# fasion-image-generator-project/discogan_modernized

Measured on AMD Instinct MI355X. Metric: images/sec per DiscoGAN train step, higher is better.
Workload: dtype f32x3; 1 GPU; tops2hanbok discogan image_size=512 batch_size=32 per GPU (BASELINE configs[3]); D,G,G cycle, fwd+bwd+Adam, dead backward work skipped; fp32-accurate conv products on the bf16 matrix path: every fp32 operand carried as three bf16 planes (24 significand bits), exact bf16 x bf16 products, fp32 accumulation (no operand rounding); image_size=512, global_batch=32, parallelism=dp1, hipgraph=True, hip_streams=2, allreduce_overlap=False

## Files before the change

discogan_modernized_amd/csrc/edge.hip:

```cpp
#include "dg_common.h"
#include <type_traits>

__device__ float dg_zero_edge[64];

__device__ __forceinline__ int tap_of(int parity, int d) {
    if (parity == 0) return d == 0 ? 1 : (d == -1 ? 3 : -1);
    return d == 0 ? 2 : (d == 1 ? 0 : -1);
}

__global__ __launch_bounds__(256) void c3_dgrad_valu_kernel(const float* __restrict__ dy, const float* __restrict__ w,
                                                            float* __restrict__ dx, int N, int H, int W, int K,
                                                            int lgHo, int lgWo, int act) {
    const int Ho = H >> 1, Wo = W >> 1;
    const long nquad = (long)N * Ho * Wo;
    const long q = (long)blockIdx.x * 256 + threadIdx.x;
    if (q >= nquad) return;
    const int b = (int)(q & (Wo - 1)), a = (int)((q >> lgWo) & (Ho - 1)), n = (int)(q >> (lgWo + lgHo));
    float acc[3][2][2];
#pragma unroll
    for (int c = 0; c < 3; ++c) acc[c][0][0] = acc[c][0][1] = acc[c][1][0] = acc[c][1][1] = 0.f;
    const float* base = dy + ((long)(n * Ho + a) * Wo + b) * K;
    for (int k0 = 0; k0 < K; k0 += 4) {
        f32x4 g[3][3];
#pragma unroll
// ... 260 lines not shown
                }
        } else if constexpr (MF16) {
#pragma unroll
            for (int st = 0; st < 2; ++st)
#pragma unroll
                for (int g = 0; g < 2; ++g)
#pragma unroll
                    for (int blk = 0; blk < 3; ++blk)
                        acc[g][blk] = __builtin_amdgcn_mfma_f32_16x16x32_bf16(__builtin_bit_cast(bf16x8_d, areg[S][g][st]), breg16[blk][st],
                                                                              acc[g][blk], 0, 0, 0);
        } else
#pragma unroll
        for (int s = 0; s < 16; ++s)
#pragma unroll
            for (int g = 0; g < 2; ++g)
#pragma unroll
                for (int blk = 0; blk < 3; ++blk)
                {
                    float av;
                    if constexpr (IN16) {
                        const float fv = areg[S][g][s >> 3][(s >> 1) & 3];
                        const unsigned wv = __float_as_uint(fv);
                        av = __builtin_bit_cast(float, (s & 1) ? (wv & 0xffff0000u) : (wv << 16));
                    } else {
                        av = areg[S][g][s >> 2][s & 3];
                    }
                    acc[g][blk] = __builtin_amdgcn_mfma_f32_16x16x4f32(av, breg[blk][s], acc[g][blk], 0, 0, 0);
                }
        __syncthreads();
#pragma unroll
        for (int g = 0; g < 2; ++g)
#pragma unroll
            for (int blk = 0; blk < 3; ++blk)
#pragma unroll
                for (int j = 0; j < 4; ++j) Ps[((wave + 4 * g) * CS_PC + 4 * kq + j) * CS_LDP + blk * 16 + p] = acc[g][blk][j];
        __syncthreads();
        for (int e = tid; e < 3 * 2 * CS_TR * 2 * CS_TC; e += 256) {
            const int xx = e % (2 * CS_TC), yy = (e / (2 * CS_TC)) % (2 * CS_TR), c = e / (4 * CS_TR * CS_TC);
            const int y = 2 * a0 + yy, x = 2 * b0 + xx;
            const int ph = yy & 1, pw = xx & 1, la = (yy >> 1) + 1, lb = (xx >> 1) + 1;
            const int ra2 = la - 1 + 2 * ph, rr1 = 1 + ph, rr2 = 3 - 3 * ph;
            const int cb2 = lb - 1 + 2 * pw, ss1 = 1 + pw, ss2 = 3 - 3 * pw;
            const float* pc = Ps + c * 16;
            float v = pc[(la * CS_PC + lb) * CS_LDP + rr1 * 4 + ss1] + pc[(la * CS_PC + cb2) * CS_LDP + rr1 * 4 + ss2] +
                      pc[(ra2 * CS_PC + lb) * CS_LDP + rr2 * 4 + ss1] + pc[(ra2 * CS_PC + cb2) * CS_LDP + rr2 * 4 + ss2];
            if (act == DG_ACT_SIGMOID) v = 1.f / (1.f + expf(-v));
            if (y < H && x < W) dx[((long)(n * 3 + c) * H + y) * W + x] = v;
        }
        apply_act(S ^ 1);
    };
    for (int t = blockIdx.x; t < ntiles; t += 2 * gridDim.x) {
        tile(std::integral_constant<int, 0>{}, t);
        if (t + (int)gridDim.x < ntiles) tile(std::integral_constant<int, 1>{}, t + gridDim.x);
    }
}

extern "C" size_t dg_c3_dgrad_workspace_bytes(int K) { return K == CD_K ? (size_t)CD_NK * 16 * sizeof(float) : 0; }
static int c3_dgrad_run(int groups, const float* const* dy_nhwc, int dy_bf16, const float* const* w, float* const* dx_nchw, int N, int H, int W, int K,
                        int act, void* ws, size_t ws_bytes, dg_stream_t stream, const void* act_out = nullptr, float slope = 0.f);
extern "C" int dg_conv4x4s2_c3_dgrad(const float* dy_nhwc, const float* w, float* dx_nchw, int N, int H, int W, int K,
                                     int act, void* ws, size_t ws_bytes, dg_stream_t stream) {
    return c3_dgrad_run(1, &dy_nhwc, 0, &w, &dx_nchw, N, H, W, K, act, ws, ws_bytes, stream);
}
extern "C" int dg_conv4x4s2_c3_dgrad_t(const void* dy_nhwc, int dy_bf16, const float* w, float* dx_nchw, int N, int H, int W, int K,
                                       int act, void* ws, size_t ws_bytes, dg_stream_t stream) {
    const float* dyp = (const float*)dy_nhwc;
    return c3_dgrad_run(1, &dyp, dy_bf16, &w, &dx_nchw, N, H, W, K, act, ws, ws_bytes, stream);
}
extern "C" int dg_conv4x4s2_c3_dgrad_p(const void* dy_nhwc, int dy_bf16, const float* w, float* dx_nchw, int N, int H, int W, int K,
                                       int act, int prec, void* ws, size_t ws_bytes, dg_stream_t stream) {
    DG_CHECK_ARG(prec >= DG_PREC_DEFAULT && prec <= DG_PREC_F32X3, "dg_conv4x4s2_c3_dgrad_p: prec=%d", prec);
    DgPrecScope scope(prec);
    const float* dyp = (const float*)dy_nhwc;
    return c3_dgrad_run(1, &dyp, dy_bf16, &w, &dx_nchw, N, H, W, K, act, ws, ws_bytes, stream);
}
static bool c3_dgrad_scatter_fits(int N, int H, int W, int K, int dy_bf16) {
    return K == CD_K && N >= 1 && (long)N * (H / 2) * (W / 2) * CD_K * (dy_bf16 ? 2 : 4) < (1L << 31);
}
extern "C" int dg_c3_dgrad_act_ok(int N, int H, int W, int K, int dy_bf16) {
    return c3_dgrad_scatter_fits(N, H, W, K, dy_bf16) && dg_get_option(DG_OPT_KT) != 16 ? 1 : 0;
}
extern "C" int dg_conv4x4s2_c3_dgrad_act_p(const void* dy_nhwc, int dy_bf16, const void* act_out, int in_act, float slope, const float* w, float* dx_nchw,
                                           int N, int H, int W, int K, int act, int prec, void* ws, size_t ws_bytes, dg_stream_t stream) {
    DG_CHECK_ARG(prec >= DG_PREC_DEFAULT && prec <= DG_PREC_F32X3, "dg_conv4x4s2_c3_dgrad_act_p: prec=%d", prec);
    DG_CHECK_ARG(act_out && in_act == DG_ACT_LEAKY, "dg_conv4x4s2_c3_dgrad_act_p: needs the saved output of a fused LeakyReLU (in_act=%d)", in_act);
    DG_CHECK_ARG(dg_c3_dgrad_act_ok(N, H, W, K, dy_bf16), "dg_conv4x4s2_c3_dgrad_act_p: the fused form is the scatter kernel (K == 64, dy under 2^31 bytes, option kt != 16)");
    DgPrecScope scope(prec);
    const float* dyp = (const float*)dy_nhwc;
    return c3_dgrad_run(1, &dyp, dy_bf16, &w, &dx_nchw, N, H, W, K, act, ws, ws_bytes, stream, act_out, slope);
}
extern "C" int dg_conv4x4s2_c3_dgrad_g(int groups, const float* const* dy_nhwc, const float* const* w, float* const* dx_nchw, int N, int H, int W, int K,
                                       int act, int prec, dg_stream_t stream) {
    DG_CHECK_ARG(groups >= 1 && groups <= DG_MAX_GROUPS && dy_nhwc && w && dx_nchw, "dg_conv4x4s2_c3_dgrad_g: bad group / null table");
    DG_CHECK_ARG(prec >= DG_PREC_DEFAULT && prec <= DG_PREC_F32X3, "dg_conv4x4s2_c3_dgrad_g: prec=%d", prec);
    DG_CHECK_ARG(K == CD_K && dg_get_option(DG_OPT_KT) != 16, "dg_conv4x4s2_c3_dgrad_g: the grouped form is the scatter kernel (K == 64)");
    DgPrecScope scope(prec);
    return c3_dgrad_run(groups, dy_nhwc, 0, w, dx_nchw, N, H, W, K, act, nullptr, 0, stream);
}
static int c3_dgrad_run(int groups, const float* const* dy_tab, int dy_bf16, const float* const* w_tab, float* const* dx_tab, int N, int H, int W, int K,
                        int act, void* ws, size_t ws_bytes, dg_stream_t stream, const void* act_out, float slope) {
    DG_CHECK_ARG(act_out == nullptr || groups == 1, "dg_conv4x4s2_c3_dgrad: the fused activation backward takes one problem");
    for (int i = 0; i < groups; ++i) DG_CHECK_ARG(dy_tab[i] && w_tab[i] && dx_tab[i], "dg_conv4x4s2_c3_dgrad: null pointer");
    const float* dy_nhwc = dy_tab[0];
    const float* w = w_tab[0];
    float* dx_nchw = dx_tab[0];
    DG_CHECK_ARG(!dy_bf16 || (K == CD_K && dg_get_option(DG_OPT_KT) != 16), "dg_conv4x4s2_c3_dgrad_t: a bf16 dy needs K == 64 (scatter form)");
    DG_CHECK_ARG(N >= 1 && K >= 4 && K % 4 == 0, "dg_conv4x4s2_c3_dgrad: bad N/K (%d,%d)", N, K);
    DG_CHECK_ARG(dg_is_pow2(H) && dg_is_pow2(W) && H >= 2 && W >= 2, "dg_conv4x4s2_c3_dgrad: H,W must be powers of two");
    DG_CHECK_ARG(act == DG_ACT_NONE || act == DG_ACT_SIGMOID, "dg_conv4x4s2_c3_dgrad: bad act %d", act);
    DG_CHECK_ARG((long)N * 3 * H * W < (1L << 31), "dg_conv4x4s2_c3_dgrad: tensor too large");
    hipStream_t st = (hipStream_t)stream;
    const int Ho = H / 2, Wo = W / 2;
    if (c3_dgrad_scatter_fits(N, H, W, K, dy_bf16)) {
        if (dg_get_option(DG_OPT_KT) != 16) {
            const int tiles_r = (Ho + CS_TR - 1) / CS_TR, tiles_c = (Wo + CS_TC - 1) / CS_TC;
            const long ntiles = (long)N * tiles_r * tiles_c;
            DG_CHECK_ARG(ntiles < (1L << 30), "dg_conv4x4s2_c3_dgrad: too many tiles");
            const dim3 grid((unsigned)(ntiles < 512 ? ntiles : 512), groups);
            const DgPtrs pd = dg_ptrs((const void* const*)dy_tab, groups), pw = dg_ptrs((const void* const*)w_tab, groups),
                         px = dg_ptrs((const void* const*)dx_tab, groups);
            const DgPtrs pa = dg_ptrs1(act_out ? act_out : (const void*)dy_tab[0]);
            const unsigned dyb = (unsigned)((long)N * Ho * Wo * CD_K * (dy_bf16 ? 2 : 4));
#define C3_SCATTER(...) hipLaunchKernelGGL((c3_dgrad_scatter_kernel<__VA_ARGS__>), grid, dim3(256), 0, st, pd, pw, px, N, H, W, act, tiles_r, tiles_c, (int)ntiles, dyb, pa, slope)
            if (dy_bf16 && dg_cur_prec() == 1) {
                if (act_out) C3_SCATTER(true, true, false, true); else C3_SCATTER(true, true);
            } else if (dy_bf16) {
                if (act_out) C3_SCATTER(true, false, false, true); else C3_SCATTER(true, false);
            } else if (dg_cur_prec() == 2) {
                if (act_out) C3_SCATTER(false, false, true, true); else C3_SCATTER(false, false, true);
            } else {
                if (act_out) C3_SCATTER(false, false, false, true); else C3_SCATTER(false, false);
            }
#undef C3_SCATTER
            DG_CHECK_LAUNCH("c3_dgrad_scatter");
            return DG_OK;
        }
        DG_CHECK_ARG(groups == 1 && !act_out, "dg_conv4x4s2_c3_dgrad: the gather form takes one problem and no fused activation backward");
        DG_CHECK_ARG(!dy_bf16, "dg_conv4x4s2_c3_dgrad: the gather form reads an fp32 dy (a bf16 dy needs the scatter form)");
        const int tiles_r = (Ho + CD_TR - 1) / CD_TR, tiles_c = (Wo + CD_TC - 1) / CD_TC;
        const long ntiles = (long)N * tiles_r * tiles_c;
        DG_CHECK_ARG(ntiles < (1L << 31), "dg_conv4x4s2_c3_dgrad: too many tiles");
        if (ws == nullptr || ws_bytes < dg_c3_dgrad_workspace_bytes(K))
            return dg_fail(DG_ERR_WORKSPACE, "dg_conv4x4s2_c3_dgrad: workspace %zu < %zu", ws_bytes, dg_c3_dgrad_workspace_bytes(K));
        hipLaunchKernelGGL(c3_wq_build_kernel, dim3((CD_NK * 16 + 255) / 256), dim3(256), 0, st, w, (float*)ws);
        DG_CHECK_LAUNCH("c3_wq_build");
        const int grid = (int)(ntiles < 512 ? ntiles : 512);
        hipLaunchKernelGGL(c3_dgrad_mfma_kernel, dim3(grid), dim3(256), 0, st, dy_nhwc, (const float*)ws, dx_nchw, N, H, W, act,
                           tiles_r, tiles_c, (int)ntiles);
        DG_CHECK_LAUNCH("c3_dgrad_mfma");
        return DG_OK;
    }
    DG_CHECK_ARG(groups == 1 && !act_out, "dg_conv4x4s2_c3_dgrad: the VALU form takes one problem and no fused activation backward");
    DG_CHECK_ARG(!dy_bf16, "dg_conv4x4s2_c3_dgrad: the VALU form reads an fp32 dy (a bf16 dy of %ld bytes is past the scatter form's 2^31)",
                 (long)N * Ho * Wo * K * 2);
    const long nquad = (long)N * Ho * Wo;
    hipLaunchKernelGGL(c3_dgrad_valu_kernel, dim3((unsigned)((nquad + 255) / 256)), dim3(256), 0, st, dy_nhwc, w,
                       dx_nchw, N, H, W, K, dg_ilog2(Ho), dg_ilog2(Wo), act);
    DG_CHECK_LAUNCH("c3_dgrad_valu");
    return DG_OK;
}

#define CF_K 64
#define CF_S 24
template <int ACT, bool OUT16>
__global__ __launch_bounds__(256, 2) void c3_fwd_mfma_kernel(const DgPtrs xs, const DgPtrs ws_, const DgPtrs ys, int N, int H, int W, int lgHo, int lgWo,
                                                             long npix, int ngroups, float slope, int xbytes) {
    const float* __restrict__ x = dg_pick<const float>(xs, blockIdx.y);
    const float* __restrict__ w = dg_pick<const float>(ws_, blockIdx.y);
    float* __restrict__ y = dg_pick<float>(ys, blockIdx.y);
    const int lane = threadIdx.x & 63;
    const int p = lane & 31, h = lane >> 5;
    const int Ho = H >> 1, Wo = W >> 1;
    const int wave = blockIdx.x * 4 + (threadIdx.x >> 6), nwaves = gridDim.x * 4;
    const float* const zp = dg_zero_edge;
    __shared__ float wS[CF_K * 49];
    for (int e = threadIdx.x; e < CF_K * 48; e += 256) wS[(e / 48) * 49 + e % 48] = w[e];
    __syncthreads();
    float wb[2][CF_S];
#pragma unroll
    for (int nb = 0; nb < 2; ++nb)
#pragma unroll
        for (int s = 0; s < CF_S; ++s) {
// ... 524 lines not shown
        u32x4_w ev, od;
#pragma unroll
        for (int u = 0; u < 4; ++u) {
            ev[u] = __builtin_amdgcn_perm(w8[2 * u + 1], w8[2 * u], 0x05040100u);
            od[u] = __builtin_amdgcn_perm(w8[2 * u + 1], w8[2 * u], 0x07060302u);
        }
        fa[0] = __builtin_bit_cast(bf16x8_w, ev);
        fa[1] = __builtin_bit_cast(bf16x8_w, od);
#pragma unroll
        for (int jn = 0; jn < 2; ++jn) {
            f32x8_w t8;
#pragma unroll
            for (int t = 0; t < 8; ++t) t8[t] = fb[set][jn][t];
            fbv[jn] = __builtin_convertvector(t8, bf16x8_w);
        }
#pragma unroll
        for (int i = 0; i < 2; ++i)
#pragma unroll
            for (int jn = 0; jn < 2; ++jn) acc[i][jn] = __builtin_amdgcn_mfma_f32_32x32x16_bf16(fa[i], fbv[jn], acc[i][jn], 0, 0, 0);
    };
    load_batch(0, p_begin);
    for (long p0 = p_begin; p0 < p_end; p0 += 32) {
        load_batch(1, p0 + 16);
        mma_batch(0);
        load_batch(0, p0 + 32);
        mma_batch(1);
    }
    __shared__ float slabS[4][64 * 48];
#pragma unroll
    for (int i = 0; i < 2; ++i)
#pragma unroll
        for (int r = 0; r < 16; ++r) {
            const int rho = (r & 3) + 8 * (r >> 2) + 4 * lh;
            const int k = 2 * rho + i;
#pragma unroll
            for (int jn = 0; jn < 2; ++jn) {
                const int j = jn * 32 + l31;
                if (j < 48) slabS[wave][k * 48 + j] = acc[i][jn][r];
            }
        }
    __syncthreads();
    float* slab = part + ((long)blockIdx.x * K + kg * 64) * 48;
    for (int e = tid; e < 64 * 48; e += 256) slab[e] = ((slabS[0][e] + slabS[1][e]) + slabS[2][e]) + slabS[3][e];
}

#define CWL_WOMAX 256
template <typename F>
__device__ __forceinline__ void c3_static_for4(F&& f) {
    f(std::integral_constant<int, 0>{});
    f(std::integral_constant<int, 1>{});
    f(std::integral_constant<int, 2>{});
    f(std::integral_constant<int, 3>{});
}
template <bool FACT, bool X3 = false>
__global__ __launch_bounds__(256, X3 ? 1 : 2) void c3_wgrad_lds_kernel(const DgPtrs dys, const DgPtrs xs, const DgPtrs parts, int N, int H, int W, int K,
                                                              long npix, int rows_per_wg, const DgPtrs act_outs, float slope) {
    const float* __restrict__ dy = dg_pick<const float>(dys, blockIdx.z);
    const float* __restrict__ x = dg_pick<const float>(xs, blockIdx.z);
    float* __restrict__ part = dg_pick<float>(parts, blockIdx.z);
    const float* __restrict__ act_out = dg_pick<const float>(act_outs, blockIdx.z);
    constexpr int ROWE = CWL_WOMAX + 8;
    typedef typename std::conditional<X3, float, __bf16>::type ET;
    __shared__ __attribute__((aligned(16))) ET img[2][4][12][ROWE];
    const int tid = threadIdx.x, lane = tid & 63, wave = tid >> 6;
    const int l31 = lane & 31, lh = lane >> 5;
    const int Ho = H >> 1, Wo = W >> 1;
    const int kg = blockIdx.y;
    f32x16 acc[2][2];
#pragma unroll
    for (int i = 0; i < 2; ++i)
#pragma unroll
        for (int j = 0; j < 2; ++j)
#pragma unroll
            for (int r = 0; r < 16; ++r) acc[i][j][r] = 0.f;
    int jrow[2], jarr[2];
    bool jok[2];
#pragma unroll
    for (int jn = 0; jn < 2; ++jn) {
        const int j = jn * 32 + l31;
        jok[jn] = j < 48;
        const int jj = jok[jn] ? j : 0;
        jarr[jn] = jj & 3;
        jrow[jn] = (jj >> 4) * 4 + ((jj >> 2) & 3);
    }
    const int nrows = N * Ho;
    const int u0 = blockIdx.x * rows_per_wg, u1 = min(nrows, u0 + rows_per_wg);
    constexpr int BIG = 0x40000000;
    constexpr int EB = X3 ? 4 : 2;
    const __amdgpu_buffer_rsrc_t rdy = __builtin_amdgcn_make_buffer_rsrc((void*)dy, 0, (int)(npix * K * EB), 0x00020000);
    const __amdgpu_buffer_rsrc_t rao = __builtin_amdgcn_make_buffer_rsrc((void*)(FACT ? act_out : dy), 0, (int)(npix * K * EB), 0x00020000);
    auto bload = [](const __amdgpu_buffer_rsrc_t& r, int off) -> unsigned {
        return (unsigned)__builtin_amdgcn_raw_buffer_load_b32(r, off, 0, 0);
    };
    typedef float f32x2_w __attribute__((ext_vector_type(2)));
    auto bload2 = [](const __amdgpu_buffer_rsrc_t& r, int off) -> f32x2_w {
        return __builtin_bit_cast(f32x2_w, __builtin_amdgcn_raw_buffer_load_b64(r, off, 0, 0));
    };
    const int wq = W >> 2, chunks = 12 * wq;
    f32x4 sv[6];
    auto stage_load = [&](int u) {
        const int n = u / Ho, oy = u - n * Ho;
#pragma unroll
        for (int k = 0; k < 6; ++k) {
            const int e = tid + 256 * k;
            const int rowi = e / wq, m = e - rowi * wq;
            const int c = rowi >> 2, r = rowi & 3;
            const int iy = 2 * oy - 1 + r;
            sv[k] = (f32x4){0.f, 0.f, 0.f, 0.f};
            if (e < chunks && (unsigned)iy < (unsigned)H) sv[k] = *(const f32x4*)(x + ((long)(n * 3 + c) * H + iy) * W + 4 * m);
        }
    };
    auto stage_store = [&](int st) {
#pragma unroll
        for (int k = 0; k < 6; ++k) {
            const int e = tid + 256 * k;
            if (e >= chunks) continue;
            const int rowi = e / wq, m = e - rowi * wq;
            typedef ET etx4_s __attribute__((ext_vector_type(4)));
            typedef ET etx2_s __attribute__((ext_vector_type(2)));
            const etx4_s b = __builtin_convertvector(sv[k], etx4_s);
            ET* E = &img[st][1][rowi][0];
            ET* O = &img[st][2][rowi][0];
            ET* O0 = &img[st][0][rowi][0];
            ET* E1 = &img[st][3][rowi][0];
            *(etx2_s*)(E + 2 * m) = (etx2_s){b[0], b[2]};
            *(etx2_s*)(O + 2 * m) = (etx2_s){b[1], b[3]};
            O0[2 * m + 1] = b[1];
            if (2 * m + 2 < Wo) O0[2 * m + 2] = b[3];
            E1[2 * m] = b[2];
            if (m > 0) E1[2 * m - 1] = b[0];
            if (m == 0) O0[0] = (ET)0.f;
            if (2 * m + 2 == Wo) E1[Wo - 1] = (ET)0.f;
        }
    };
    constexpr int NSET = X3 ? 4 : 2;
    unsigned wa[2][X3 ? 1 : 8], wo[2][(FACT && !X3) ? 8 : 1];
    f32x2_w fa2[NSET][X3 ? 8 : 1], fo2[NSET][(FACT && X3) ? 8 : 1];
    const int nbatch = Wo >> 4;
    auto load_a = [&](int set, int u, int b) {
#pragma unroll
        for (int t = 0; t < 8; ++t) {
            const int pp = u * Wo + 16 * b + 8 * lh + t;
            const int aoff = (u < u1 && b < nbatch) ? (pp * K + kg * 64 + 2 * l31) * EB : BIG;
            if constexpr (X3) {
                fa2[set][t] = bload2(rdy, aoff);
                if constexpr (FACT) fo2[set][t] = bload2(rao, aoff);
            } else {
                wa[set][t] = bload(rdy, aoff);
                if constexpr (FACT) wo[set][t] = bload(rao, aoff);
            }
        }
    };
    typedef __bf16 bf16x8_l __attribute__((ext_vector_type(8)));
    typedef unsigned u32x4_l __attribute__((ext_vector_type(4)));
    typedef float f32x8_l __attribute__((ext_vector_type(8)));
    auto split8 = [](const f32x8_l& v, bf16x8_l* pl) {
        pl[0] = __builtin_convertvector(v, bf16x8_l);
        const f32x8_l r1 = v - __builtin_convertvector(pl[0], f32x8_l);
        pl[1] = __builtin_convertvector(r1, bf16x8_l);
        pl[2] = __builtin_convertvector(r1 - __builtin_convertvector(pl[1], f32x8_l), bf16x8_l);
    };
    auto mma_x3 = [&](int set, int st, int b) {
        if constexpr (X3) {
            f32x8_l a0, a1;
#pragma unroll
            for (int t = 0; t < 8; ++t) {
                f32x2_w v = fa2[set][t];
                if constexpr (FACT) {
                    const f32x2_w o = fo2[set][t];
                    v[0] = o[0] > 0.f ? v[0] : v[0] * slope;
                    v[1] = o[1] > 0.f ? v[1] : v[1] * slope;
                }
                a0[t] = v[0];
                a1[t] = v[1];
            }
            bf16x8_l pa0[3], pa1[3];
            split8(a0, pa0);
            split8(a1, pa1);
            constexpr int PA[6] = {2, 0, 1, 1, 0, 0}, PB[6] = {0, 2, 1, 0, 1, 0};
#pragma unroll
            for (int jn = 0; jn < 2; ++jn) {
                const float* src = (const float*)&img[st][jarr[jn]][jrow[jn]][16 * b + 8 * lh];
                const f32x4 lo = *(const f32x4*)src, hi = *(const f32x4*)(src + 4);
                f32x8_l bv = {lo[0], lo[1], lo[2], lo[3], hi[0], hi[1], hi[2], hi[3]};
                if (!jok[jn]) bv = (f32x8_l){0.f, 0.f, 0.f, 0.f, 0.f, 0.f, 0.f, 0.f};
                bf16x8_l pb[3];
                split8(bv, pb);
#pragma unroll
                for (int q = 0; q < 6; ++q) {
                    acc[0][jn] = __builtin_amdgcn_mfma_f32_32x32x16_bf16(pa0[PA[q]], pb[PB[q]], acc[0][jn], 0, 0, 0);
                    acc[1][jn] = __builtin_amdgcn_mfma_f32_32x32x16_bf16(pa1[PA[q]], pb[PB[q]], acc[1][jn], 0, 0, 0);
                }
            }
        }
    };
    auto mma = [&](int set, int st, int b) {
        if constexpr (X3) {
            mma_x3(set, st, b);
            return;
        } else {
        unsigned w8[8];
#pragma unroll
        for (int t = 0; t < 8; ++t) {
            unsigned wv = wa[set][t];
            if constexpr (FACT) {
                const unsigned ov = wo[set][t];
                float a0 = __builtin_bit_cast(float, wv << 16), a1 = __builtin_bit_cast(float, wv & 0xffff0000u);
                a0 = __builtin_bit_cast(float, ov << 16) > 0.f ? a0 : a0 * slope;
                a1 = __builtin_bit_cast(float, ov & 0xffff0000u) > 0.f ? a1 : a1 * slope;
                typedef __bf16 bf16x2_l __attribute__((ext_vector_type(2)));
                typedef float f32x2_l __attribute__((ext_vector_type(2)));
                wv = __builtin_bit_cast(unsigned, __builtin_convertvector((f32x2_l){a0, a1}, bf16x2_l));
            }
            w8[t] = wv;
        }
        u32x4_l ev, od;
#pragma unroll
        for (int q = 0; q < 4; ++q) {
            ev[q] = __builtin_amdgcn_perm(w8[2 * q + 1], w8[2 * q], 0x05040100u);
            od[q] = __builtin_amdgcn_perm(w8[2 * q + 1], w8[2 * q], 0x07060302u);
        }
        const bf16x8_l fa0 = __builtin_bit_cast(bf16x8_l, ev), fa1 = __builtin_bit_cast(bf16x8_l, od);
        bf16x8_l fb[2];
#pragma unroll
        for (int jn = 0; jn < 2; ++jn) {
            fb[jn] = *(const bf16x8_l*)(const void*)&img[st][jarr[jn]][jrow[jn]][16 * b + 8 * lh];
            if (!jok[jn]) fb[jn] = __builtin_bit_cast(bf16x8_l, (u32x4_l){0u, 0u, 0u, 0u});
        }
#pragma unroll
        for (int jn = 0; jn < 2; ++jn) {
            acc[0][jn] = __builtin_amdgcn_mfma_f32_32x32x16_bf16(fa0, fb[jn], acc[0][jn], 0, 0, 0);
            acc[1][jn] = __builtin_amdgcn_mfma_f32_32x32x16_bf16(fa1, fb[jn], acc[1][jn], 0, 0, 0);
        }
        }
    };
    for (int e = tid; e < 2 * 4 * 12 * ROWE; e += 256) (&img[0][0][0][0])[e] = (ET)0.f;
    __syncthreads();
    if (u0 < u1) {
        stage_load(u0);
        stage_store(0);
    }
    load_a(0, u0, wave);
    __syncthreads();
    if constexpr (X3) {
        if (nbatch == 16) {
            load_a(1, u0, wave + 4);
            load_a(2, u0, wave + 8);
            for (int u = u0; u < u1; ++u) {
                const int st = (u - u0) & 1;
                if (u + 1 < u1) stage_load(u + 1);
                c3_static_for4([&](auto J_) {
                    constexpr int J = decltype(J_)::value;
                    constexpr int JN = (J + 3) & 3;
                    load_a(JN, J + 3 >= 4 ? u + 1 : u, wave + 4 * JN);
                    mma_x3(J, st, wave + 4 * J);
                });
                if (u + 1 < u1) stage_store(st ^ 1);
                __syncthreads();
            }
        }
    }
    bool odd = false;
    auto item = [&](auto S_, int u, int b, int st) {
        constexpr int S = decltype(S_)::value;
        const bool last = b + 4 >= nbatch;
        load_a(S ^ 1, last ? u + 1 : u, last ? wave : b + 4);
        mma(S, st, b);
    };
    for (int u = (X3 && nbatch == 16) ? u1 : u0; u < u1; ++u) {
        const int st = (u - u0) & 1;
        if (u + 1 < u1) stage_load(u + 1);
        for (int b = wave; b < nbatch; b += 4) {
            if (odd) item(std::integral_constant<int, 1>{}, u, b, st);
            else item(std::integral_constant<int, 0>{}, u, b, st);
            odd = !odd;
        }
        if (u + 1 < u1) stage_store(st ^ 1);
        __syncthreads();
    }
    static_assert(sizeof(img) >= 4 * 64 * 48 * sizeof(float), "slab reduction lives in the image stages");
    float (*slabS)[64 * 48] = (float (*)[64 * 48]) & img[0][0][0][0];
#pragma unroll
    for (int i = 0; i < 2; ++i)
#pragma unroll
        for (int r = 0; r < 16; ++r) {
            const int rho = (r & 3) + 8 * (r >> 2) + 4 * lh;
            const int k = 2 * rho + i;
#pragma unroll
            for (int jn = 0; jn < 2; ++jn) {
                const int j = jn * 32 + l31;
                if (j < 48) slabS[wave][k * 48 + j] = acc[i][jn][r];
            }
        }
    __syncthreads();
    float* slab = part + ((long)blockIdx.x * K + kg * 64) * 48;
    for (int e = tid; e < 64 * 48; e += 256) slab[e] = ((slabS[0][e] + slabS[1][e]) + slabS[2][e]) + slabS[3][e];
}

__global__ __launch_bounds__(256) void c3_wgrad_reduce_kernel(const DgPtrs parts, const DgPtrs dws, int nslabs, int total, int accumulate) {
    const float* __restrict__ part = dg_pick<const float>(parts, blockIdx.y);
    float* __restrict__ dw = dg_pick<float>(dws, blockIdx.y);
    __shared__ float red[16][17];
    const int el = threadIdx.x & 15, sl = threadIdx.x >> 4;
    const int e = blockIdx.x * 16 + el;
    float s = 0.f;
    if (e < total)
        for (int b = sl; b < nslabs; b += 16) s += part[(long)b * total + e];
    red[sl][el] = s;
    __syncthreads();
    if (sl == 0 && e < total) {
#pragma unroll
        for (int j = 1; j < 16; ++j) s += red[j][el];
        if (accumulate) s += dw[e];
        dw[e] = s;
    }
}

static void c3_wgrad_plan(long npix, int* nb, int* ppw) {
    const int unit = 4 * CW_B;
    long per = (npix + 2047) / 2048;
    per = (per + unit - 1) / unit * unit;
    if (per < unit) per = unit;
    *ppw = (int)per;
    const long nwaves = (npix + per - 1) / per;
    *nb = (int)((nwaves + 3) / 4);
}
extern "C" size_t dg_c3_wgrad_workspace_bytes(int N, int H, int W, int K) {
    const long npix = (long)N * (H / 2) * (W / 2);
    int nb, ppw;
    c3_wgrad_plan(npix, &nb, &ppw);
    return (size_t)nb * K * 48 * sizeof(float);
// ... 39 lines not shown
    DG_CHECK_ARG(share >= 1 && groups % share == 0, "dg_conv4x4s2_c3_wgrad_g: share=%d", share);
    DG_CHECK_ARG(prec >= DG_PREC_DEFAULT && prec <= DG_PREC_F32X3, "dg_conv4x4s2_c3_wgrad_g: prec=%d", prec);
    DG_CHECK_ARG(act == DG_ACT_NONE || ((act == DG_ACT_LEAKY || act == DG_ACT_RELU) && act_out_nhwc),
                 "dg_conv4x4s2_c3_wgrad_g: act %d needs the saved activation outputs (LeakyReLU / ReLU only)", act);
    const float* none[DG_MAX_GROUPS] = {nullptr, nullptr, nullptr, nullptr};
    DgPrecScope scope(prec);
    return c3_wgrad_run("dg_conv4x4s2_c3_wgrad_g", groups, share, dy_nhwc, act == DG_ACT_NONE ? none : act_out_nhwc, act, act == DG_ACT_RELU ? 0.f : slope,
                        x_nchw, dw, N, H, W, K, accumulate, ws, ws_bytes, stream);
}
static int c3_wgrad_reduce_g(int groups, int share, void* const* ws_tab, float* const* dw_tab, int nb, int total, int accumulate, hipStream_t st) {
    const int nout = groups / share;
    for (int j = 0; j < share; ++j) {
        const void* pp[DG_MAX_GROUPS];
        const void* dd[DG_MAX_GROUPS];
        for (int z = 0; z < nout; ++z) { pp[z] = ws_tab[z * share + j]; dd[z] = dw_tab[z * share + j]; }
        hipLaunchKernelGGL(c3_wgrad_reduce_kernel, dim3((total + 15) / 16, nout), dim3(256), 0, st, dg_ptrs(pp, nout), dg_ptrs(dd, nout), nb, total,
                           (accumulate || j > 0) ? 1 : 0);
        DG_CHECK_LAUNCH("c3_wgrad_reduce");
    }
    return DG_OK;
}
static int c3_wgrad_run(const char* who, int groups, int share, const float* const* dy_tab, const float* const* ao_tab, int act, float slope,
                        const float* const* x_tab, float* const* dw_tab, int N, int H, int W, int K, int accumulate, void* const* ws_tab, size_t ws_bytes,
                        dg_stream_t stream, int io_bf16) {
    for (int i = 0; i < groups; ++i) DG_CHECK_ARG(dy_tab[i] && x_tab[i] && dw_tab[i], "%s: null pointer", who);
    for (int i = 0; i < groups; ++i) DG_CHECK_ARG(dw_tab[i] == dw_tab[i / share * share], "%s: problems of one share set must name the same dw", who);
    const float* dy_nhwc = dy_tab[0];
    const float* x_nchw = x_tab[0];
    const float* act_out = ao_tab[0];
    void* ws = ws_tab[0];
    for (int i = 0; i < groups; ++i) DG_CHECK_ARG((ao_tab[i] != nullptr) == (act_out != nullptr), "%s: activation outputs for all problems or none", who);
    DG_CHECK_ARG(N >= 1 && K >= 64 && K % 64 == 0, "%s: K=%d must be a multiple of 64", who, K);
    DG_CHECK_ARG(dg_is_pow2(H) && dg_is_pow2(W) && H >= 2 && W >= 2, "%s: H,W must be powers of two", who);
    DG_CHECK_ARG((long)N * 3 * H * W < (1L << 31), "%s: tensor too large", who);
    const long npix = (long)N * (H / 2) * (W / 2);
    int nb, ppw;
    c3_wgrad_plan(npix, &nb, &ppw);
    const size_t need = (size_t)nb * K * 48 * sizeof(float);
    for (int i = 0; i < groups; ++i)
        if (ws_tab[i] == nullptr || ws_bytes < need) return dg_fail(DG_ERR_WORKSPACE, "%s: workspace %zu < %zu", who, ws_bytes, need);
    hipStream_t st = (hipStream_t)stream;
    const bool buf = npix * K * 4 < (1L << 30) && (long)N * 3 * H * W * 4 < (1L << 30) && dg_get_option(DG_OPT_POINTER_PATH) == 0;
    const bool fact = act_out != nullptr;
    const DgPtrs pdy = dg_ptrs((const void* const*)dy_tab, groups), px = dg_ptrs((const void* const*)x_tab, groups),
                 pws = dg_ptrs((const void* const*)ws_tab, groups), pao = dg_ptrs((const void* const*)ao_tab, groups);
    const dim3 grid(nb, K / 64, groups);
#define CW_LAUNCH(B, F)                                                                                                  \
    hipLaunchKernelGGL((c3_wgrad_mfma_kernel<B, F>), grid, dim3(256), 0, st, pdy, px, pws, N, H, W, \
                       K, dg_ilog2(H / 2), dg_ilog2(W / 2), npix, ppw, pao, slope)
    if (io_bf16 && !buf) return dg_fail(DG_ERR_INVALID, "%s: bf16 operands need tensors < 1 GiB", who);
    if (!io_bf16 && buf && dg_cur_prec() == 2 && W >= 256 && W / 2 <= CWL_WOMAX && dg_get_option(DG_OPT_KT) != 16) {
        const int nrows = N * (H / 2);
        const int rpw = (nrows + nb - 1) / nb;
        if (fact)
            hipLaunchKernelGGL((c3_wgrad_lds_kernel<true, true>), grid, dim3(256), 0, st, pdy, px, pws, N, H, W, K, npix, rpw, pao, slope);
        else
            hipLaunchKernelGGL((c3_wgrad_lds_kernel<false, true>), grid, dim3(256), 0, st, pdy, px, pws, N, H, W, K, npix, rpw, pao, slope);
        DG_CHECK_LAUNCH("c3_wgrad_lds_x3");
        return c3_wgrad_reduce_g(groups, share, ws_tab, dw_tab, nb, K * 48, accumulate, st);
    }
    if (io_bf16 && dg_cur_prec() == 1 && W >= 32 && W / 2 <= CWL_WOMAX && dg_get_option(DG_OPT_KT) != 16) {
        const int nrows = N * (H / 2);
        const int rpw = (nrows + nb - 1) / nb;
        if (fact)
            hipLaunchKernelGGL(c3_wgrad_lds_kernel<true>, grid, dim3(256), 0, st, pdy, px, pws, N, H, W, K, npix, rpw, pao, slope);
        else
            hipLaunchKernelGGL(c3_wgrad_lds_kernel<false>, grid, dim3(256), 0, st, pdy, px, pws, N, H, W, K, npix, rpw, pao, slope);
    } else if (io_bf16 && dg_cur_prec() == 1) {
        DG_CHECK_ARG(groups == 1, "%s: this kernel takes one problem", who);
        if (fact)
            hipLaunchKernelGGL(c3_wgrad_bf16mfma_kernel<true>, dim3(nb, K / 64), dim3(256), 0, st, dy_nhwc, x_nchw, (float*)ws, N, H, W,
                               K, dg_ilog2(H / 2), dg_ilog2(W / 2), npix, ppw, act_out, slope);
        else
            hipLaunchKernelGGL(c3_wgrad_bf16mfma_kernel<false>, dim3(nb, K / 64), dim3(256), 0, st, dy_nhwc, x_nchw, (float*)ws, N, H, W,
                               K, dg_ilog2(H / 2), dg_ilog2(W / 2), npix, ppw, act_out, slope);
    } else if (io_bf16 && fact) {
        hipLaunchKernelGGL((c3_wgrad_mfma_kernel<true, true, true>), grid, dim3(256), 0, st, pdy, px, pws, N, H, W,
                           K, dg_ilog2(H / 2), dg_ilog2(W / 2), npix, ppw, pao, slope);
    } else if (io_bf16) {
        hipLaunchKernelGGL((c3_wgrad_mfma_kernel<true, false, true>), grid, dim3(256), 0, st, pdy, px, pws, N, H, W,
                           K, dg_ilog2(H / 2), dg_ilog2(W / 2), npix, ppw, pao, slope);
    } else if (buf && fact) CW_LAUNCH(true, true);
    else if (buf) CW_LAUNCH(true, false);
    else if (fact) CW_LAUNCH(false, true);
    else CW_LAUNCH(false, false);
#undef CW_LAUNCH
    DG_CHECK_LAUNCH("c3_wgrad_mfma");
    return c3_wgrad_reduce_g(groups, share, ws_tab, dw_tab, nb, K * 48, accumulate, st);
}
```

Baseline: 298.2 images/s.

## Add banded f32x3 C=3 dgrad kernel and deepen f32x3 wgrad LDS pipeline

Adds a new f32x3 dgrad kernel for the 3-channel 4x4 stride-2 conv. It walks row bands per column strip, keeps the three bf16 weight planes in registers, and reuses overlapping output rows through a rotating three-slot LDS buffer, in place of the generic scatter tile path. The f32x3 wgrad LDS kernel gets a compact two-array padded image layout, 2-wave occupancy, and a deeper prefetch schedule for W/2=256 that splits staging loads and stores across the MFMA iterations. The aim is less redundant dy traffic and LDS use and better latency hiding, at the cost of more complex indexing and register pressure.

```diff
diff --git a/discogan_modernized_amd/csrc/edge.hip b/discogan_modernized_amd/csrc/edge.hip
--- a/discogan_modernized_amd/csrc/edge.hip
+++ b/discogan_modernized_amd/csrc/edge.hip
@@ -336,6 +336,162 @@
     for (int t = blockIdx.x; t < ntiles; t += 2 * gridDim.x) {
         tile(std::integral_constant<int, 0>{}, t);
         if (t + (int)gridDim.x < ntiles) tile(std::integral_constant<int, 1>{}, t + gridDim.x);
+    }
+}
+
+#define CB_WC 64
+#define CB_FC (CB_WC - 2)
+#define CB_BAND 17
+template <bool FACT>
+__global__ __launch_bounds__(256, 2) void c3_dgrad_band_x3_kernel(const DgPtrs dys, const DgPtrs ws_, const DgPtrs dxs, int N, int H, int W, int act,
+                                                                  int band_u, int nbands, int tiles_c, int nitems, unsigned dybytes, const DgPtrs aos,
+                                                                  float slope) {
+    const float* __restrict__ dy = dg_pick<const float>(dys, blockIdx.y);
+    const float* __restrict__ w = dg_pick<const float>(ws_, blockIdx.y);
+    float* __restrict__ dx = dg_pick<float>(dxs, blockIdx.y);
+    typedef __bf16 bf16x8_d __attribute__((ext_vector_type(8)));
+    typedef float f32x8_d __attribute__((ext_vector_type(8)));
+    __shared__ __attribute__((aligned(16))) float Ps[3 * CB_WC * CS_LDP];
+    const int tid = threadIdx.x, lane = tid & 63, wave = tid >> 6;
+    const int p = lane & 15, kq = lane >> 4;
+    const int Ho = H >> 1, Wo = W >> 1;
+    bf16x8_d breg3[3][3][2];
+    auto split8 = [](const f32x8_d& v, bf16x8_d* pl) {
+        pl[0] = __builtin_convertvector(v, bf16x8_d);
+        const f32x8_d r1 = v - __builtin_convertvector(pl[0], f32x8_d);
+        pl[1] = __builtin_convertvector(r1, bf16x8_d);
+        pl[2] = __builtin_convertvector(r1 - __builtin_convertvector(pl[1], f32x8_d), bf16x8_d);
+    };
+#pragma unroll
+    for (int blk = 0; blk < 3; ++blk)
+#pragma unroll
+        for (int st = 0; st < 2; ++st) {
+            f32x8_d t;
+#pragma unroll
+            for (int j = 0; j < 8; ++j) t[j] = w[(32 * st + 8 * kq + j) * 48 + blk * 16 + p];
+            bf16x8_d pl[3];
+            split8(t, pl);
+#pragma unroll
+            for (int q = 0; q < 3; ++q) breg3[q][blk][st] = pl[q];
+        }
+    const __amdgpu_buffer_rsrc_t rdy = __builtin_amdgcn_make_buffer_rsrc((void*)dy, 0, (int)dybytes, 0x00020000);
+    const __amdgpu_buffer_rsrc_t rao = __builtin_amdgcn_make_buffer_rsrc((void*)(FACT ? dg_pick<const float>(aos, blockIdx.y) : dy), 0, (int)dybytes, 0x00020000);
+    constexpr int OOR = (int)0x80000000;
+    f32x4 areg[2][2][4];
+    f32x4 oreg[FACT ? 2 : 1][4];
+    auto apply_act = [&](int set) {
+        if constexpr (FACT) {
+#pragma unroll
+            for (int g = 0; g < 2; ++g)
+#pragma unroll
+                for (int j = 0; j < 4; ++j)
+#pragma unroll
+                    for (int e = 0; e < 4; ++e) {
+                        const float d = areg[set][g][j][e];
+                        areg[set][g][j][e] = oreg[g][j][e] > 0.f ? d : d * slope;
+                    }
+        }
+    };
+    auto steps_of = [&](int t) {
+        const int r0 = ((t / tiles_c) % nbands) * band_u, r1 = min(r0 + band_u, Ho + 1);
+        return (r1 - r0 + 2) >> 1;
+    };
+    auto fetch = [&](int t, int s, int set) {
+        const int tc = t % tiles_c, band = (t / tiles_c) % nbands, n = t / (tiles_c * nbands);
+        const int r0 = band * band_u, rend = min(r0 + band_u, Ho);
+        const int b = tc * CB_FC - 1 + 16 * wave + p;
+#pragma unroll
+        for (int g = 0; g < 2; ++g) {
+            const int a = r0 - 1 + 2 * s + g;
+            const bool ok = t < nitems && a >= 0 && a < rend && (unsigned)b < (unsigned)Wo;
+            const int off = ok ? (((n * Ho + a) * Wo + b) * CD_K + 8 * kq) * 4 : OOR;
+#pragma unroll
+            for (int j = 0; j < 4; ++j) {
+                const int o = off + 128 * (j >> 1) + 16 * (j & 1);
+                areg[set][g][j] = __builtin_bit_cast(f32x4, __builtin_amdgcn_raw_buffer_load_b128(rdy, o, 0, 0));
+                if constexpr (FACT) oreg[g][j] = __builtin_bit_cast(f32x4, __builtin_amdgcn_raw_buffer_load_b128(rao, o, 0, 0));
+            }
+        }
+    };
+    const int oxx = tid & 127, ohf = tid >> 7;
+    const int olb = ((oxx >> 1) + 1) * CS_LDP + 1 + (oxx & 1), ocb = ((oxx >> 1) + 2 * (oxx & 1)) * CS_LDP + 3 - 3 * (oxx & 1);
+    int t = blockIdx.x, s = 0, ns = steps_of(t), cs = 2;
+    fetch(t, 0, 0);
+    apply_act(0);
+    auto step = [&](auto SB) {
+        constexpr int S = decltype(SB)::value;
+        int t2 = t, s2 = s + 1;
+        if (s2 == ns) {
+            t2 = t + gridDim.x;
+            s2 = 0;
+        }
+        fetch(t2, s2, S ^ 1);
+        const int tc = t % tiles_c, band = (t / tiles_c) % nbands, n = t / (tiles_c * nbands);
+        const int r0 = band * band_u, r1 = min(r0 + band_u, Ho + 1), b0 = tc * CB_FC;
+        const int a = r0 + 2 * s;
+        if (s == 0) cs = 2;
+        const int sl1 = cs == 2 ? 0 : cs + 1, sl2 = cs == 0 ? 2 : cs - 1;
+        const bool wave_on = b0 - 1 + 16 * wave <= Wo;
+        f32x4 acc[2][3];
+#pragma unroll
+        for (int g = 0; g < 2; ++g)
+#pragma unroll
+            for (int blk = 0; blk < 3; ++blk) acc[g][blk] = (f32x4){0.f, 0.f, 0.f, 0.f};
+        if (wave_on) {
+            constexpr int PA[6] = {2, 0, 1, 1, 0, 0}, PB[6] = {0, 2, 1, 0, 1, 0};
+#pragma unroll
+            for (int st = 0; st < 2; ++st)
+#pragma unroll
+                for (int g = 0; g < 2; ++g) {
+                    const f32x4 v0 = areg[S][g][2 * st], v1 = areg[S][g][2 * st + 1];
+                    bf16x8_d apl[3];
+                    split8((f32x8_d){v0[0], v0[1], v0[2], v0[3], v1[0], v1[1], v1[2], v1[3]}, apl);
+#pragma unroll
+                    for (int blk = 0; blk < 3; ++blk)
+#pragma unroll
+                        for (int q = 0; q < 6; ++q)
+                            acc[g][blk] = __builtin_amdgcn_mfma_f32_16x16x32_bf16(apl[PA[q]], breg3[PB[q]][blk][st], acc[g][blk], 0, 0, 0);
+                }
+        }
+        __syncthreads();
+        if (wave_on) {
+#pragma unroll
+            for (int g = 0; g < 2; ++g)
+#pragma unroll
+                for (int blk = 0; blk < 3; ++blk)
+#pragma unroll
+                    for (int j = 0; j < 4; ++j)
+                        Ps[((g ? sl2 : sl1) * CB_WC + 16 * wave + 4 * kq + j) * CS_LDP + blk * 16 + p] = acc[g][blk][j];
+        }
+        __syncthreads();
+        const int ylim = min(H, 2 * r1 - 1);
+        const int x = 2 * b0 + oxx;
+        if (oxx < 2 * CB_FC && x < W) {
+#pragma unroll
+            for (int i = 0; i < 6; ++i) {
+                const int cy = 2 * i + ohf, c = cy >> 2, yy = cy & 3;
+                const int y = 2 * a - 3 + yy;
+                if ((s == 0 && yy < 2) || (unsigned)y >= (unsigned)ylim) continue;
+                const int ph = (yy + 1) & 1, la = (yy + 1) >> 1;
+                const int ra2 = la - 1 + 2 * ph, rr1 = 1 + ph, rr2 = 3 - 3 * ph;
+                const int s1 = cs + la >= 3 ? cs + la - 3 : cs + la, s2r = cs + ra2 >= 3 ? cs + ra2 - 3 : cs + ra2;
+                const float* p1 = Ps + s1 * (CB_WC * CS_LDP) + c * 16 + rr1 * 4;
+                const float* p2 = Ps + s2r * (CB_WC * CS_LDP) + c * 16 + rr2 * 4;
+                float v = p1[olb] + p1[ocb] + p2[olb] + p2[ocb];
+                if (act == DG_ACT_SIGMOID) v = 1.f / (1.f + expf(-v));
+                dx[((long)(n * 3 + c) * H + y) * W + x] = v;
+            }
+        }
+        apply_act(S ^ 1);
+        cs = sl2;
+        if (s2 == 0) ns = steps_of(t2);
+        t = t2;
+        s = s2;
+    };
+    while (t < nitems) {
+        step(std::integral_constant<int, 0>{});
+        if (t >= nitems) break;
+        step(std::integral_constant<int, 1>{});
     }
 }
 
@@ -411,7 +567,13 @@
             } else if (dy_bf16) {
                 if (act_out) C3_SCATTER(true, false, false, true); else C3_SCATTER(true, false);
             } else if (dg_cur_prec() == 2) {
-                if (act_out) C3_SCATTER(false, false, true, true); else C3_SCATTER(false, false, true);
+                const int units = Ho + 1, band_u = CB_BAND < (units | 1) ? CB_BAND : (units | 1);
+                const int nbands = (units + band_u - 1) / band_u, strips = (Wo + CB_FC - 1) / CB_FC;
+                const long nitems = (long)N * nbands * strips;
+                const dim3 bgrid((unsigned)(nitems < 512 ? nitems : 512), groups);
+#define C3_BAND(F) hipLaunchKernelGGL((c3_dgrad_band_x3_kernel<F>), bgrid, dim3(256), 0, st, pd, pw, px, N, H, W, act, band_u, nbands, strips, (int)nitems, dyb, pa, slope)
+                if (act_out) C3_BAND(true); else C3_BAND(false);
+#undef C3_BAND
             } else {
                 if (act_out) C3_SCATTER(false, false, false, true); else C3_SCATTER(false, false);
             }
@@ -1042,16 +1204,19 @@
     f(std::integral_constant<int, 2>{});
     f(std::integral_constant<int, 3>{});
 }
-template <bool FACT, bool X3 = false>
-__global__ __launch_bounds__(256, X3 ? 1 : 2) void c3_wgrad_lds_kernel(const DgPtrs dys, const DgPtrs xs, const DgPtrs parts, int N, int H, int W, int K,
+template <bool FACT, bool X3 = false, bool DEEP = false>
+__global__ __launch_bounds__(256, 2) void c3_wgrad_lds_kernel(const DgPtrs dys, const DgPtrs xs, const DgPtrs parts, int N, int H, int W, int K,
                                                               long npix, int rows_per_wg, const DgPtrs act_outs, float slope) {
     const float* __restrict__ dy = dg_pick<const float>(dys, blockIdx.z);
     const float* __restrict__ x = dg_pick<const float>(xs, blockIdx.z);
     float* __restrict__ part = dg_pick<float>(parts, blockIdx.z);
     const float* __restrict__ act_out = dg_pick<const float>(act_outs, blockIdx.z);
+    if constexpr (DEEP) W = 2 * CWL_WOMAX;
     constexpr int ROWE = CWL_WOMAX + 8;
+    constexpr int NARR = X3 ? 2 : 4;
+    constexpr int XPAD = 4;
     typedef typename std::conditional<X3, float, __bf16>::type ET;
-    __shared__ __attribute__((aligned(16))) ET img[2][4][12][ROWE];
+    __shared__ __attribute__((aligned(16))) ET img[2][NARR][12][ROWE];
     const int tid = threadIdx.x, lane = tid & 63, wave = tid >> 6;
     const int l31 = lane & 31, lh = lane >> 5;
     const int Ho = H >> 1, Wo = W >> 1;
@@ -1072,6 +1237,7 @@
         const int jj = jok[jn] ? j : 0;
         jarr[jn] = jj & 3;
         jrow[jn] = (jj >> 4) * 4 + ((jj >> 2) & 3);
+        if constexpr (X3) jarr[jn] = (((jj & 1) ? 0 : 12) + jrow[jn]) * ROWE + ((jj & 3) == 0 ? XPAD - 1 : (jj & 3) == 2 ? XPAD : (jj & 3) == 3 ? 1 : 0);
     }
     const int nrows = N * Ho;
     const int u0 = blockIdx.x * rows_per_wg, u1 = min(nrows, u0 + rows_per_wg);
@@ -1088,10 +1254,12 @@
     };
     const int wq = W >> 2, chunks = 12 * wq;
     f32x4 sv[6];
-    auto stage_load = [&](int u) {
+    constexpr std::integral_constant<int, 0> k_0{};
+    constexpr std::integral_constant<int, 6> k_6{};
+    auto stage_load = [&](int u, auto K0_, auto K1_) {
         const int n = u / Ho, oy = u - n * Ho;
 #pragma unroll
-        for (int k = 0; k < 6; ++k) {
+        for (int k = decltype(K0_)::value; k < decltype(K1_)::value; ++k) {
             const int e = tid + 256 * k;
             const int rowi = e / wq, m = e - rowi * wq;
             const int c = rowi >> 2, r = rowi & 3;
@@ -1100,30 +1268,35 @@
             if (e < chunks && (unsigned)iy < (unsigned)H) sv[k] = *(const f32x4*)(x + ((long)(n * 3 + c) * H + iy) * W + 4 * m);
         }
     };
-    auto stage_store = [&](int st) {
-#pragma unroll
-        for (int k = 0; k < 6; ++k) {
+    auto stage_store = [&](int st, auto K0_, auto K1_) {
+#pragma unroll
+        for (int k = decltype(K0_)::value; k < decltype(K1_)::value; ++k) {
             const int e = tid + 256 * k;
             if (e >= chunks) continue;
             const int rowi = e / wq, m = e - rowi * wq;
             typedef ET etx4_s __attribute__((ext_vector_type(4)));
             typedef ET etx2_s __attribute__((ext_vector_type(2)));
             const etx4_s b = __builtin_convertvector(sv[k], etx4_s);
-            ET* E = &img[st][1][rowi][0];
-            ET* O = &img[st][2][rowi][0];
-            ET* O0 = &img[st][0][rowi][0];
-            ET* E1 = &img[st][3][rowi][0];
-            *(etx2_s*)(E + 2 * m) = (etx2_s){b[0], b[2]};
-            *(etx2_s*)(O + 2 * m) = (etx2_s){b[1], b[3]};
-            O0[2 * m + 1] = b[1];
-            if (2 * m + 2 < Wo) O0[2 * m + 2] = b[3];
-            E1[2 * m] = b[2];
-            if (m > 0) E1[2 * m - 1] = b[0];
-            if (m == 0) O0[0] = (ET)0.f;
-            if (2 * m + 2 == Wo) E1[Wo - 1] = (ET)0.f;
-        }
-    };
-    constexpr int NSET = X3 ? 4 : 2;
+            if constexpr (X3) {
+                *(etx2_s*)(&img[st][0][rowi][0] + 2 * m) = (etx2_s){b[0], b[2]};
+                *(etx2_s*)(&img[st][1][rowi][0] + XPAD + 2 * m) = (etx2_s){b[1], b[3]};
+            } else {
+                ET* E = &img[st][1][rowi][0];
+                ET* O = &img[st][2][rowi][0];
+                ET* O0 = &img[st][0][rowi][0];
+                ET* E1 = &img[st][3][rowi][0];
+                *(etx2_s*)(E + 2 * m) = (etx2_s){b[0], b[2]};
+                *(etx2_s*)(O + 2 * m) = (etx2_s){b[1], b[3]};
+                O0[2 * m + 1] = b[1];
+                if (2 * m + 2 < Wo) O0[2 * m + 2] = b[3];
+                E1[2 * m] = b[2];
+                if (m > 0) E1[2 * m - 1] = b[0];
+                if (m == 0) O0[0] = (ET)0.f;
+                if (2 * m + 2 == Wo) E1[Wo - 1] = (ET)0.f;
+            }
+        }
+    };
+    constexpr int NSET = DEEP ? (FACT ? 2 : 4) : 2;
     unsigned wa[2][X3 ? 1 : 8], wo[2][(FACT && !X3) ? 8 : 1];
     f32x2_w fa2[NSET][X3 ? 8 : 1], fo2[NSET][(FACT && X3) ? 8 : 1];
     const int nbatch = Wo >> 4;
@@ -1170,9 +1343,10 @@
             constexpr int PA[6] = {2, 0, 1, 1, 0, 0}, PB[6] = {0, 2, 1, 0, 1, 0};
 #pragma unroll
             for (int jn = 0; jn < 2; ++jn) {
-                const float* src = (const float*)&img[st][jarr[jn]][jrow[jn]][16 * b + 8 * lh];
-                const f32x4 lo = *(const f32x4*)src, hi = *(const f32x4*)(src + 4);
-                f32x8_l bv = {lo[0], lo[1], lo[2], lo[3], hi[0], hi[1], hi[2], hi[3]};
+                const float* src = (const float*)&img[st][0][0][0] + jarr[jn] + 16 * b + 8 * lh;
+                f32x8_l bv;
+#pragma unroll
+                for (int t = 0; t < 8; ++t) bv[t] = src[t];
                 if (!jok[jn]) bv = (f32x8_l){0.f, 0.f, 0.f, 0.f, 0.f, 0.f, 0.f, 0.f};
                 bf16x8_l pb[3];
                 split8(bv, pb);
@@ -1224,32 +1398,49 @@
         }
         }
     };
-    for (int e = tid; e < 2 * 4 * 12 * ROWE; e += 256) (&img[0][0][0][0])[e] = (ET)0.f;
+    for (int e = tid; e < 2 * NARR * 12 * ROWE; e += 256) (&img[0][0][0][0])[e] = (ET)0.f;
     __syncthreads();
     if (u0 < u1) {
-        stage_load(u0);
-        stage_store(0);
+        stage_load(u0, k_0, k_6);
+        stage_store(0, k_0, k_6);
     }
     load_a(0, u0, wave);
     __syncthreads();
-    if constexpr (X3) {
-        if (nbatch == 16) {
-            load_a(1, u0, wave + 4);
-            load_a(2, u0, wave + 8);
-            for (int u = u0; u < u1; ++u) {
+    static_assert(!DEEP || X3, "the deep loop is the f32x3 form's");
+    if constexpr (DEEP) {
+        {
+            constexpr int D = NSET - 1;
+#pragma unroll
+            for (int d = 1; d < D; ++d) load_a(d, u0, wave + 4 * d);
+            auto row = [&](auto Q0_, int u) {
+                constexpr int Q0 = decltype(Q0_)::value;
                 const int st = (u - u0) & 1;
-                if (u + 1 < u1) stage_load(u + 1);
                 c3_static_for4([&](auto J_) {
                     constexpr int J = decltype(J_)::value;
-                    constexpr int JN = (J + 3) & 3;
-                    load_a(JN, J + 3 >= 4 ? u + 1 : u, wave + 4 * JN);
-                    mma_x3(J, st, wave + 4 * J);
+                    constexpr int JN = (J + D) & 3;
+                    constexpr std::integral_constant<int, 3 * (J >> 1)> K0{};
+                    constexpr std::integral_constant<int, 3 * (J >> 1) + 3> K1{};
+                    if ((J & 1) == 0 && u + 1 < u1) stage_load(u + 1, K0, K1);
+                    load_a((Q0 + J + D) % NSET, J + D >= 4 ? u + 1 : u, wave + 4 * JN);
+                    mma_x3((Q0 + J) % NSET, st, wave + 4 * J);
+                    if ((J & 1) == 1 && u + 1 < u1) stage_store(st ^ 1, K0, K1);
                 });
-                if (u + 1 < u1) stage_store(st ^ 1);
                 __syncthreads();
-            }
-        }
-    }
+            };
+            int q0 = 0;
+            for (int u = u0; u < u1; ++u) {
+                if constexpr (NSET == 3) {
+                    if (q0 == 0) row(std::integral_constant<int, 0>{}, u);
+                    else if (q0 == 1) row(std::integral_constant<int, 1>{}, u);
+                    else row(std::integral_constant<int, 2>{}, u);
+                    q0 = q0 == 2 ? 0 : q0 + 1;
+                } else {
+                    row(std::integral_constant<int, 0>{}, u);
+                }
+            }
+        }
+    }
+    if constexpr (!DEEP) {
     bool odd = false;
     auto item = [&](auto S_, int u, int b, int st) {
         constexpr int S = decltype(S_)::value;
@@ -1257,16 +1448,17 @@
         load_a(S ^ 1, last ? u + 1 : u, last ? wave : b + 4);
         mma(S, st, b);
     };
-    for (int u = (X3 && nbatch == 16) ? u1 : u0; u < u1; ++u) {
+    for (int u = u0; u < u1; ++u) {
         const int st = (u - u0) & 1;
-        if (u + 1 < u1) stage_load(u + 1);
+        if (u + 1 < u1) stage_load(u + 1, k_0, k_6);
         for (int b = wave; b < nbatch; b += 4) {
             if (odd) item(std::integral_constant<int, 1>{}, u, b, st);
             else item(std::integral_constant<int, 0>{}, u, b, st);
             odd = !odd;
         }
-        if (u + 1 < u1) stage_store(st ^ 1);
+        if (u + 1 < u1) stage_store(st ^ 1, k_0, k_6);
         __syncthreads();
+    }
     }
     static_assert(sizeof(img) >= 4 * 64 * 48 * sizeof(float), "slab reduction lives in the image stages");
     float (*slabS)[64 * 48] = (float (*)[64 * 48]) & img[0][0][0][0];
@@ -1412,10 +1604,13 @@
     if (!io_bf16 && buf && dg_cur_prec() == 2 && W >= 256 && W / 2 <= CWL_WOMAX && dg_get_option(DG_OPT_KT) != 16) {
         const int nrows = N * (H / 2);
         const int rpw = (nrows + nb - 1) / nb;
-        if (fact)
-            hipLaunchKernelGGL((c3_wgrad_lds_kernel<true, true>), grid, dim3(256), 0, st, pdy, px, pws, N, H, W, K, npix, rpw, pao, slope);
-        else
-            hipLaunchKernelGGL((c3_wgrad_lds_kernel<false, true>), grid, dim3(256), 0, st, pdy, px, pws, N, H, W, K, npix, rpw, pao, slope);
+        const bool deep = W / 2 == 256;
+#define CWL_X3(F, D) hipLaunchKernelGGL((c3_wgrad_lds_kernel<F, true, D>), grid, dim3(256), 0, st, pdy, px, pws, N, H, W, K, npix, rpw, pao, slope)
+        if (fact && deep) CWL_X3(true, true);
+        else if (fact) CWL_X3(true, false);
+        else if (deep) CWL_X3(false, true);
+        else CWL_X3(false, false);
+#undef CWL_X3
         DG_CHECK_LAUNCH("c3_wgrad_lds_x3");
         return c3_wgrad_reduce_g(groups, share, ws_tab, dw_tab, nb, K * 48, accumulate, st);
     }
```

Result: no change. 299.6 images/s (median of 6 runs) (+0.5%).
